# Cyan4973/FiniteStateEntropy

Measured on NVIDIA H100. Metric: encode+decode GB/s (uncompressed) per GPU on 32 KB blocks; bit-exact vs ref, higher is better.
Workload: dtype u8

## Files before the change

### finitestateentropy_b200/csrc/huf_encode.cu

```cuda
#include <cstdlib>
#include <mutex>
#include <vector>
#include "common.cuh"
#include "launch_util.cuh"
#include "fse_dev.cuh"
#include "sink_dev.cuh"
#include "huf_build_dev.cuh"

namespace fseb {
namespace hufe {

constexpr unsigned FULL = 0xFFFFFFFFu;

struct __align__(16) Plan {
    u32 ctable[256];
    u8  header[136];
    u32 hSize;
    u32 state;
    u32 total;
    u32 streamOff[4];
    u32 streamBytes[4];
};

constexpr int PLAN_WARPS = 8;
struct PlanWarp {
    u32   count4[4][256];
    u32   count[256];
    HNode nodes[2 * 256 + 2];
    u32   ctable[256];
    u32   firstVal[32];
    u8    lenOf[256];
    alignas(4) u8 header[136];
};
static_assert(sizeof(HNode) * (2 * 256 + 2) >= 384 * sizeof(u32), "header scratch must fit in the node array");
__device__ __forceinline__ u32 seg_count(const PlanWarp& w, u32 k, u32 i) { return w.count4[k][i]; }

__device__ __forceinline__ void warp_hist_range(u32* cnt, const u8* s, u32 begin, u32 end, unsigned lane)
{
    u32 i = begin;
    u32 const head = min(end, (u32)((begin + 15) & ~15u));
    bool const vec = ((reinterpret_cast<u64>(s) & 15) == 0);
    if (vec) {
        for (u32 k = i + lane; k < head; k += 32) atomicAdd(&cnt[s[k]], 1u);
        i = head;
        u32 const nvec = (end - i) / 16;
        const uint4* const gv = reinterpret_cast<const uint4*>(s + i);
        for (u32 v0 = 0; v0 < nvec; v0 += 128) {
            uint4 x[4];
            #pragma unroll
            for (int h = 0; h < 4; h++) { u32 const vi = v0 + 32 * h + lane; x[h] = (vi < nvec) ? __ldg(gv + vi) : make_uint4(0, 0, 0, 0); }
            #pragma unroll
            for (int h = 0; h < 4; h++) {
                if (v0 + 32 * h + lane >= nvec) continue;
                u32 const wd[4] = { x[h].x, x[h].y, x[h].z, x[h].w };
                #pragma unroll
                for (int k = 0; k < 4; k++) {
                    u32 const y = wd[k];
                    atomicAdd(&cnt[y & 0xFF], 1u); atomicAdd(&cnt[__byte_perm(y, 0, 0x4441)], 1u);
                    atomicAdd(&cnt[__byte_perm(y, 0, 0x4442)], 1u); atomicAdd(&cnt[y >> 24], 1u);
                }
            }
        }
        i += nvec * 16;
    }
    for (u32 k = i + lane; k < end; k += 32) atomicAdd(&cnt[s[k]], 1u);
}

__device__ __forceinline__ void warp_hist4_pipelined(u32 (*count4)[256], const u8* s, u32 n, u32 seg, unsigned lane)
{
    const uint4* const gv = reinterpret_cast<const uint4*>(s) + lane;
    u32 const B = n / 2048, perSeg = seg / 2048;
    auto load = [&](uint4 (&x)[4], u32 b) {
        #pragma unroll
        for (int h = 0; h < 4; h++) x[h] = __ldg(gv + b * 128 + 32 * h);
    };
    auto count = [&](const uint4 (&x)[4], u32 b) {
        u32* const cnt = count4[b / perSeg];
        #pragma unroll
        for (int h = 0; h < 4; h++) {
            u32 const wd[4] = { x[h].x, x[h].y, x[h].z, x[h].w };
            #pragma unroll
            for (int k = 0; k < 4; k++) {
                u32 const y = wd[k];
                atomicAdd(&cnt[y & 0xFF], 1u); atomicAdd(&cnt[__byte_perm(y, 0, 0x4441)], 1u);
                atomicAdd(&cnt[__byte_perm(y, 0, 0x4442)], 1u); atomicAdd(&cnt[y >> 24], 1u);
            }
        }
    };
    uint4 xa[4], xb[4];
    load(xa, 0);
    #pragma unroll 1
    for (u32 b = 0; b < B; b += 2) {
        if (b + 1 < B) load(xb, b + 1);
        count(xa, b);
        if (b + 2 < B) load(xa, b + 2);
        if (b + 1 < B) count(xb, b + 1);
    }
}

__global__ void __launch_bounds__(32 * PLAN_WARPS)
huf_plan_kernel(BatchGeom g, u8* __restrict__ cbuf, u64* __restrict__ csizes, const u8* __restrict__ src,
                unsigned msvReq, unsigned tlogReq, Plan* __restrict__ plans, int serialHeader)
{
    extern __shared__ __align__(16) unsigned char smem_raw[];
    PlanWarp& w = reinterpret_cast<PlanWarp*>(smem_raw)[threadIdx.x >> 5];
    unsigned const lane = threadIdx.x & 31u;
    u32 const b = blockIdx.x * PLAN_WARPS + (threadIdx.x >> 5);
    if (b >= g.nBlocks) return;
    u32 const n = block_len(g, b);
    const u8* const s = src + (u64)b * g.blockSize;
    u8* const d = cbuf + (u64)b * g.slot;
    u64 const cap = g.slot;
    Plan& P = plans[b];
#define FSEB_FINAL(v) do { if (lane == 0) { P.state = 1; csizes[b] = (v); } return; } while (0)

    if (!n) FSEB_FINAL(0);
    if (!cap) FSEB_FINAL(0);
    if (n > HUF_BLOCK_MAX) FSEB_FINAL(err(E_SRC_WRONG));
    if (tlogReq > HUF_MAX_TLOG) FSEB_FINAL(err(E_TLOG_TOO_LARGE));
    if (msvReq > HUF_MAX_SV) FSEB_FINAL(err(E_MSV_TOO_LARGE));
    unsigned const msvDecl = msvReq ? msvReq : HUF_MAX_SV;
    unsigned huffLog = tlogReq ? tlogReq : HUF_DEF_TLOG;

    u32 const seg = (n + 3) / 4;
    for (u32 i = lane; i < 4 * 256; i += 32) (&w.count4[0][0])[i] = 0;
    __syncwarp();
    if ((reinterpret_cast<u64>(s) & 15) == 0 && seg % 2048 == 0 && n == 4 * seg) warp_hist4_pipelined(w.count4, s, n, seg, lane);
    else {
        #pragma unroll 1
        for (u32 k = 0; k < 4; k++) {
            u32 const beg = min(k * seg, n), end = (k < 3) ? min((k + 1) * seg, n) : n;
            warp_hist_range(w.count4[k], s, beg, end, lane);
        }
    }
    __syncwarp();
    u32 top = 0, best = 0;
    for (u32 i = lane; i < 256; i += 32) {
        u32 const c = seg_count(w, 0, i) + seg_count(w, 1, i) + seg_count(w, 2, i) + seg_count(w, 3, i);
        w.count[i] = c;
        if (c) top = i; best = c > best ? c : best;
    }
    #pragma unroll
    for (int dlt = 16; dlt; dlt >>= 1) { top = max(top, __shfl_xor_sync(FULL, top, dlt)); best = max(best, __shfl_xor_sync(FULL, best, dlt)); }
    __syncwarp();
    if (msvDecl < 255 && top > msvDecl) FSEB_FINAL(err(E_MSV_TOO_SMALL));
    if (best == n) { if (lane == 0) d[0] = s[0]; FSEB_FINAL(1); }
    if (best <= (n >> 7) + 4) FSEB_FINAL(0);
    u32 const msv = top;

    huffLog = d_optimal_tablelog(huffLog, n, msv, 1);
    {   u64 const mb = warp_huf_build_ctable(w.ctable, w.count, msv, huffLog, w.nodes, w.lenOf, w.firstVal);
        if (is_err(mb)) FSEB_FINAL(mb);
        huffLog = (u32)mb;
    }
    __syncwarp();
    u32* const wksp = reinterpret_cast<u32*>(w.nodes);
    u64 hs = 0;
    if (serialHeader) { if (lane == 0) hs = d_huf_write_ctable(w.header, cap < sizeof(w.header) ? cap : sizeof(w.header), w.ctable, msv, huffLog, wksp); hs = __shfl_sync(FULL, hs, 0); }
    else hs = warp_huf_write_ctable(w.header, cap < sizeof(w.header) ? cap : sizeof(w.header), w.ctable, msv, huffLog, wksp);
    if (is_err(hs)) FSEB_FINAL(hs);
    if (hs + 12 >= n) FSEB_FINAL(0);
    u64 const capLeft = cap - hs;
    if (capLeft < 6 + 1 + 1 + 1 + 8 || n < 12) FSEB_FINAL(0);
    u32 bits[4];
    #pragma unroll
    for (int k = 0; k < 4; k++) {
        u32 acc = 0;
        for (u32 i = lane; i <= msv; i += 32) acc += seg_count(w, k, i) * (w.ctable[i] >> 16);
        #pragma unroll
        for (int dlt = 16; dlt; dlt >>= 1) acc += __shfl_xor_sync(FULL, acc, dlt);
        bits[k] = acc;
    }
    u64 op = 6; bool fits = true;
    u32 offs[4], lens[4];
    #pragma unroll
    for (int t = 0; t < 4; t++) {
        u64 const capk = capLeft - op;
        u64 const tot = (u64)bits[t] + 1;
        if (fits && (capk <= 8 || (tot >> 3) >= capk - 8)) fits = false;
        offs[t] = (u32)(hs + op); lens[t] = (u32)((tot + 7) >> 3);
        op += lens[t];
    }
    u64 const total = hs + op;
    if (!fits || total >= (u64)n - 1) FSEB_FINAL(0);
    __syncwarp();
    for (u32 i = lane; i < 256; i += 32) P.ctable[i] = w.ctable[i];
    for (u32 i = lane; i < (u32)hs; i += 32) P.header[i] = w.header[i];
    if (lane < 4) { P.streamOff[lane] = offs[lane]; P.streamBytes[lane] = lens[lane]; }
    if (lane == 0) { P.hSize = (u32)hs; P.state = 0; P.total = (u32)total; csizes[b] = total; }
#undef FSEB_FINAL
}

constexpr int THREADS = 128;

__device__ __noinline__ void store_piece_exact(u32* gw, u32 j, uint4 v, u32 a0, u32 endByte)
{
    u32 const wd[4] = { v.x, v.y, v.z, v.w };
    u8* const pb = reinterpret_cast<u8*>(gw + j);
    for (u32 t = 0; t < 16; t++) { u32 const at = 4 * j + t; if (at >= a0 && at < endByte) pb[t] = (u8)(wd[t >> 2] >> (8 * (t & 3))); }
}

__global__ void __launch_bounds__(THREADS)
huf_emit_kernel(BatchGeom g, u8* __restrict__ cbuf, const u8* __restrict__ src, const Plan* __restrict__ plans, const u32* __restrict__ sharedCT)
{
    constexpr u32 W = 512;
    __shared__ u32 ctab[256];
    constexpr u32 WP = W + 4;
    __shared__ __align__(16) u32 winAll[4 * WP];
    int const tid = threadIdx.x;
    unsigned const lane = tid & 31u; int const k = tid >> 5;
    u32 const b = blockIdx.x;
    const Plan& P = plans[b];
    if (P.state != 0) return;
    u32 const n = block_len(g, b);
    const u8* const s = src + (u64)b * g.blockSize;
    u8* const d = cbuf + (u64)b * g.slot;
    u32 const hSize = P.hSize, total = P.total;

    {   const u32* const ct = sharedCT ? sharedCT : P.ctable;
        u32 const c0 = ct[tid], c1 = ct[tid + 128];
        ctab[tid] = (c0 >> 16) | (c0 << 8 & 0xFFFF00u); ctab[tid + 128] = (c1 >> 16) | (c1 << 8 & 0xFFFF00u);
    }
    for (u32 i = tid; i < 4 * WP; i += THREADS) winAll[i] = 0;
    for (u32 i = tid; i < hSize; i += THREADS) d[i] = P.header[i];
    if (tid < 3) { u32 const v = P.streamBytes[tid]; d[hSize + 2 * tid] = (u8)v; d[hSize + 2 * tid + 1] = (u8)(v >> 8); }
    __syncthreads();
    {
        u32 const seg = (n + 3) / 4;
        int const segBeg = (int)(k * seg);
        int const segEnd = (k < 3) ? (int)((k + 1) * seg) : (int)n;
        u32 sTab = (u32)__cvta_generic_to_shared(ctab);
        asm volatile("mov.u32 %0, %0;" : "+r"(sTab));
        u32* const win = winAll + k * WP;
        u32 sWin = (u32)__cvta_generic_to_shared(win);
        asm volatile("mov.u32 %0, %0;" : "+r"(sWin));
        u8* const gstart = d + P.streamOff[k];
        u32 const a0 = (u32)(reinterpret_cast<u64>(gstart) & 15);
        u32* const gw = reinterpret_cast<u32*>(gstart - a0);
        u32 const sBytes = (k < 3) ? P.streamBytes[k] : total - P.streamOff[3];
        u32 const endByte = a0 + sBytes;
        u32 bitpos = 8u * a0;
        u32 flushed = 0;
        auto lds32 = [&](u32 a) -> u32 { u32 v; asm volatile("ld.shared.u32 %0, [%1];" : "=r"(v) : "r"(a)); return v; };
        auto lds64 = [&](u32 o) -> uint2 { u32 const e = lds32(sTab + (o >> 1)); return make_uint2(e >> 8, e & 0xFFu); };
        auto red_or = [&](u32 a, u32 v) { asm volatile("red.shared.or.b32 [%0], %1;" :: "r"(a), "r"(v) : "memory"); };
        auto red_or3 = [&](u32 a, u32 v0, u32 v1, u32 v2) {
            asm volatile("red.shared.or.b32 [%0], %1; red.shared.or.b32 [%0+4], %2; red.shared.or.b32 [%0+8], %3;" :: "r"(a), "r"(v0), "r"(v1), "r"(v2) : "memory");
        };
        auto scan = [&](u32 held, u32& excl) -> u32 {
            u32 incl = held;
            #pragma unroll
            for (int dd = 1; dd < 32; dd <<= 1)
                asm volatile("{ .reg .pred p; .reg .u32 t; shfl.sync.up.b32 t|p, %0, %1, 0, 0xffffffff; @p add.u32 %0, %0, t; }" : "+r"(incl) : "r"(dd));
            excl = incl - held;
            return __shfl_sync(FULL, incl, 31);
        };
        auto put = [&](u32 at, u32 x0, u32 x1) {
            u32 const sh = at & 31;
            red_or3(sWin + ((at >> 3) & (4 * (W - 1))), x0 << sh, __funnelshift_l(x0, x1, sh), __funnelshift_l(x1, 0, sh));
        };
        auto put96 = [&](u32 at, u32 z0, u32 z1, u32 z2) {
            u32 const sh = at & 31;
            asm volatile("red.shared.or.b32 [%0], %1; red.shared.or.b32 [%0+4], %2; red.shared.or.b32 [%0+8], %3; red.shared.or.b32 [%0+12], %4;"
                         :: "r"(sWin + ((at >> 3) & (4 * (W - 1)))), "r"(z0 << sh), "r"(__funnelshift_l(z0, z1, sh)), "r"(__funnelshift_l(z1, z2, sh)),
                            "r"(__funnelshift_l(z2, 0, sh)) : "memory");
        };
        auto flush = [&](bool all) {
            u32 const upTo = all ? (endByte + 3) / 4 : (bitpos >> 5);
            if (!all && flushed + 128 > upTo) return;
            __syncwarp();
            while (all ? flushed < upTo : flushed + 128 <= upTo) {
                u32 const j = flushed + 4 * lane;
                if (j < upTo) {
                    u32 const i = j & (W - 1);
                    uint4 v = *reinterpret_cast<uint4*>(win + i);
                    *reinterpret_cast<uint4*>(win + i) = make_uint4(0, 0, 0, 0);
                    if (i == 0) { v.x |= win[W]; v.y |= win[W + 1]; v.z |= win[W + 2]; win[W] = 0; win[W + 1] = 0; win[W + 2] = 0; }
                    if (!all && (j != 0 || a0 == 0)) *reinterpret_cast<uint4*>(gw + j) = v;
                    else store_piece_exact(gw, j, v, a0, endByte);
                }
                flushed += 128;
            }
        };
        auto place = [&](u32 x0, u32 x1, u32 held) -> u32 {
            u32 excl; u32 const sum = scan(held, excl);
            put(bitpos + excl, x0, x1);
            return sum;
        };
        constexpr int PF = 4;
        int hiCur = segEnd;
        {
            bool const al8 = ((reinterpret_cast<u64>(s) + (u64)segEnd) & 7) == 0;
            int const nBig = al8 ? (segEnd - segBeg) / 256 : 0;
            const uint2* gq = reinterpret_cast<const uint2*>(s + segEnd) - 1 - lane;
            auto half = [&](u32 w, u32& a0, u32& a1) -> u32 {
                u32 const e0 = lds32(sTab + 4 * __byte_perm(w, 0, 0x4443)), e1 = lds32(sTab + 4 * __byte_perm(w, 0, 0x4442));
                u32 const e2 = lds32(sTab + 4 * __byte_perm(w, 0, 0x4441)), e3 = lds32(sTab + 4 * __byte_perm(w, 0, 0x4440));
                u32 const p01 = (e0 >> 8) | __funnelshift_l(0, e1 >> 8, e0), l01 = e0 + e1;
                u32 const p23 = (e2 >> 8) | __funnelshift_l(0, e3 >> 8, e2), l23 = e2 + e3;
                a0 = p01 | __funnelshift_l(0, p23, l01); a1 = __funnelshift_l(p23, 0, l01);
                return (l01 + l23) & 0xFFu;
            };
            auto merge = [&](u32 x0, u32 x1, u32 lx, u32 y0, u32 y1, u32& z0, u32& z1, u32& z2) {
                u32 const t0 = __funnelshift_l(0, y0, lx), t1 = __funnelshift_l(y0, y1, lx), t2 = __funnelshift_l(y1, 0, lx);
                bool const far = (lx & 32u) != 0;
                z0 = x0 | (far ? 0u : t0); z1 = x1 | (far ? t0 : t1); z2 = far ? t1 : t2;
            };
            auto big2 = [&](uint2 curA, uint2 curB) {
                u32 x0, x1, y0, y1, za0, za1, za2, zb0, zb1, zb2;
                u32 lx = half(curA.y, x0, x1), ly = half(curA.x, y0, y1);
                merge(x0, x1, lx, y0, y1, za0, za1, za2);
                u32 const la = lx + ly;
                lx = half(curB.y, x0, x1); ly = half(curB.x, y0, y1);
                merge(x0, x1, lx, y0, y1, zb0, zb1, zb2);
                u32 const lb = lx + ly;
                u32 excl; u32 const sum = scan(la | (lb << 16), excl);
                u32 const sumA = sum & 0xFFFFu;
                put96(bitpos + (excl & 0xFFFFu), za0, za1, za2);
                put96(bitpos + sumA + (excl >> 16), zb0, zb1, zb2);
                bitpos += sumA + (sum >> 16);
                flush(false);
            };
            constexpr int PB = 2;
            int const rounds = nBig / PB;
            uint2 bufA[PB], bufB[PB];
            #pragma unroll
            for (int i = 0; i < PB; i++) { bufA[i] = rounds > 0 ? __ldg(gq - 32 * i) : make_uint2(0, 0); bufB[i] = make_uint2(0, 0); }
            auto round = [&](uint2 (&X)[PB], uint2 (&Y)[PB], int r) {
                gq -= 32 * PB;
                uint2 const c0 = X[0], c1 = X[1];
                if (r + 1 < rounds) { Y[0] = __ldg(gq); Y[1] = __ldg(gq - 32); }
                big2(c0, c1);
            };
            int r = 0;
            #pragma unroll 1
            for (; r + 1 < rounds; r += 2) { round(bufA, bufB, r); round(bufB, bufA, r + 1); }
            if (r < rounds) round(bufA, bufB, r);
            hiCur -= 256 * rounds * PB;
        }
        bool const wordAligned = ((reinterpret_cast<u64>(s) + (u64)hiCur) & 3) == 0;
        int const nFull = wordAligned ? (hiCur - segBeg) / 128 : 0;
        {
            const u32* gp = reinterpret_cast<const u32*>(s + hiCur) - 1 - lane;
            auto group = [&](u32 o0, u32 o1, u32 o2, u32 o3) {
                uint2 const e0 = lds64(o0), e1 = lds64(o1), e2 = lds64(o2), e3 = lds64(o3);
                u32 const p01 = e0.x | (e1.x << e0.y), l01 = e0.y + e1.y;
                u32 const p23 = e2.x | (e3.x << e2.y), l23 = e2.y + e3.y;
                u32 const a0 = p01 | (p23 << l01), a1 = __funnelshift_l(p23, 0, l01);
                bitpos += place(a0, a1, l01 + l23);
                flush(false);
            };
            int const rounds = nFull / PF;
            u32 bufA[PF], bufB[PF];
            #pragma unroll
            for (int i = 0; i < PF; i++) { bufA[i] = rounds > 0 ? __ldg(gp - 32 * i) : 0u; bufB[i] = 0u; }
            auto round = [&](u32 (&X)[PF], u32 (&Y)[PF], int r) {
                gp -= 32 * PF;
                bool const more = r + 1 < rounds;
                #pragma unroll
                for (int i = 0; i < PF; i++) {
                    u32 const cur = X[i];
                    if (more) Y[i] = __ldg(gp - 32 * i);
                    group(8 * (cur >> 24), 8 * __byte_perm(cur, 0, 0x4442), 8 * __byte_perm(cur, 0, 0x4441), 8 * (cur & 0xFFu));
                }
            };
            int r = 0;
            #pragma unroll 1
            for (; r + 1 < rounds; r += 2) { round(bufA, bufB, r); round(bufB, bufA, r + 1); }
            if (r < rounds) round(bufA, bufB, r);
            for (int j = rounds * PF; j < nFull; j++) {
                u32 const cur = __ldg(reinterpret_cast<const u32*>(s + hiCur) - 1 - lane - 32 * j);
                group(8 * (cur >> 24), 8 * __byte_perm(cur, 0, 0x4442), 8 * __byte_perm(cur, 0, 0x4441), 8 * (cur & 0xFFu));
            }
        }
        {
            int const rest = hiCur - 128 * nFull;
            auto fetch = [&](int hi) -> u32 {
                int const top = hi - 4 * (int)lane;
                u32 v = 0;
                if (top - 4 >= segBeg && ((reinterpret_cast<u64>(s + top) & 3) == 0)) v = __ldg(reinterpret_cast<const u32*>(s + top - 4));
                else if (top > segBeg) {
                    #pragma unroll
                    for (int j = 0; j < 4; j++) { int const i = top - 1 - j; if (i >= segBeg) v |= (u32)s[i] << (8 * (3 - j)); }
                }
                return v;
            };
            #pragma unroll 1
            for (int hi = rest; hi > segBeg; hi -= 128) {
                u32 const cur = fetch(hi);
                int const nValid = hi - 4 * (int)lane - segBeg;
                u64 acc = 0; u32 held = 0;
                #pragma unroll
                for (int j = 0; j < 4; j++) {
                    uint2 const e = lds64(8 * ((cur >> (8 * (3 - j))) & 0xFF));
                    if (j < nValid) { acc |= (u64)e.x << held; held += e.y; }
                }
                bitpos += place((u32)acc, (u32)(acc >> 32), held);
                flush(false);
            }
        }
        if (lane == 0) red_or(sWin + 4 * ((bitpos >> 5) & (W - 1)), 1u << (bitpos & 31));
        bitpos += 1;
        flush(true);
    }
}

__global__ void __launch_bounds__(32 * PLAN_WARPS)
huf_sizes_kernel(BatchGeom g, u64* __restrict__ csizes, const u8* __restrict__ src, const u32* __restrict__ ct, Plan* __restrict__ plans)
{
    __shared__ u8 nbOf[256];
    unsigned const lane = threadIdx.x & 31u;
    for (u32 i = threadIdx.x; i < 256; i += blockDim.x) nbOf[i] = (u8)(ct[i] >> 16);
    __syncthreads();
    u32 const b = blockIdx.x * PLAN_WARPS + (threadIdx.x >> 5);
    if (b >= g.nBlocks) return;
    u32 const n = block_len(g, b);
    const u8* const s = src + (u64)b * g.blockSize;
    u64 const cap = g.slot;
    Plan& P = plans[b];
    if (cap < 6 + 1 + 1 + 1 + 8 || n < 12) { if (lane == 0) { P.state = 1; csizes[b] = 0; } return; }
    u32 const seg = (n + 3) / 4;
    u32 bits[4];
    #pragma unroll 1
    for (u32 k = 0; k < 4; k++) {
        u32 const beg = k * seg, end = (k < 3) ? (k + 1) * seg : n;
        u32 acc = 0;
        u32 i = beg + lane * 4;
        if ((reinterpret_cast<u64>(s + beg) & 3) == 0) {
            for (; i + 4 <= end; i += 128) {
                u32 const w = __ldg(reinterpret_cast<const u32*>(s + i));
                acc += nbOf[w & 0xFF] + nbOf[(w >> 8) & 0xFF] + nbOf[(w >> 16) & 0xFF] + nbOf[w >> 24];
            }
            for (u32 t = i; t < end && t < i + 4; t++) acc += nbOf[s[t]];
        } else for (u32 t = beg + lane; t < end; t += 32) acc += nbOf[s[t]];
        #pragma unroll
        for (int dlt = 16; dlt; dlt >>= 1) acc += __shfl_xor_sync(FULL, acc, dlt);
        bits[k] = acc;
    }
    u64 op = 6; bool fits = true;
    u32 offs[4], lens[4];
    #pragma unroll
    for (int t = 0; t < 4; t++) {
        u64 const capk = cap - op;
        u64 const tot = (u64)bits[t] + 1;
        if (fits && (capk <= 8 || (tot >> 3) >= capk - 8)) fits = false;
        offs[t] = (u32)op; lens[t] = (u32)((tot + 7) >> 3);
        op += lens[t];
    }
    if (!fits) { if (lane == 0) { P.state = 1; csizes[b] = 0; } return; }
    if (lane < 4) { P.streamOff[lane] = offs[lane]; P.streamBytes[lane] = lens[lane]; }
    if (lane == 0) { P.hSize = 0; P.state = 0; P.total = (u32)op; csizes[b] = op; }
}

}

cudaError_t launch_huf_encode_using_ctable(const BatchGeom& g, void* cbuf, u64* csizes, const void* src, const u32* dCTable, cudaStream_t stream)
{
    if (g.nBlocks == 0) return cudaSuccess;
    cudaError_t e;
    hufe::Plan* const plans = (hufe::Plan*)stream_scratch(2, stream, sizeof(hufe::Plan) * (size_t)g.nBlocks, &e);
    if (e != cudaSuccess) return e;
    unsigned const grid = (g.nBlocks + hufe::PLAN_WARPS - 1) / hufe::PLAN_WARPS;
    hufe::huf_sizes_kernel<<<grid, 32 * hufe::PLAN_WARPS, 0, stream>>>(g, csizes, (const u8*)src, dCTable, plans);
    hufe::huf_emit_kernel<<<g.nBlocks, hufe::THREADS, 0, stream>>>(g, (u8*)cbuf, (const u8*)src, plans, dCTable);
    return cudaGetLastError();
}

cudaError_t launch_huf_encode(const BatchGeom& g, void* cbuf, u64* csizes, const void* src,
                              unsigned msv, unsigned tlog, cudaStream_t stream)
{
    if (g.nBlocks == 0) return cudaSuccess;
    cudaError_t e;
    hufe::Plan* plans = nullptr;
    static int asyncScratch = -1;
    if (asyncScratch < 0) { const char* const v = getenv("FSEB200_SCRATCH_ASYNC"); asyncScratch = (v && atoi(v) == 1) ? 1 : 0; }
    size_t const need = sizeof(hufe::Plan) * (size_t)g.nBlocks;
    if (asyncScratch) e = cudaMallocAsync((void**)&plans, need, stream);
    else {
        struct Slot { int dev; cudaStream_t s; void* p; size_t cap; };
        static std::mutex mu; static std::vector<Slot> slots;
        std::lock_guard<std::mutex> lock(mu);
        int dev = 0; cudaGetDevice(&dev);
        Slot* hit = nullptr;
        for (auto& sl : slots) if (sl.s == stream && sl.dev == dev) { hit = &sl; break; }
        if (!hit) { slots.push_back(Slot{ dev, stream, nullptr, 0 }); hit = &slots.back(); }
        e = cudaSuccess;
        if (hit->cap < need) {
            if (hit->p) { cudaStreamSynchronize(stream); cudaFree(hit->p); hit->p = nullptr; hit->cap = 0; }
            e = cudaMalloc(&hit->p, need);
            if (e == cudaSuccess) hit->cap = need;
        }
        plans = (hufe::Plan*)hit->p;
    }
    if (e != cudaSuccess) return e;
    static int serialHeader = -1;
    if (serialHeader < 0) { const char* const v = getenv("FSEB200_HUF_SERIAL_HEADER"); serialHeader = (v && atoi(v) == 1) ? 1 : 0; }
    static u32 const subBatch = [] { const char* const v = getenv("FSEB200_HUF_ENC_SUBBATCH"); long n = v ? atol(v) : 0; return (u32)(n < 0 ? 0 : n); }();
    size_t const smem = sizeof(hufe::PlanWarp) * hufe::PLAN_WARPS;
    static SmemOptIn optin;
    e = optin.ensure(hufe::huf_plan_kernel, current_device(), (int)smem);
    if (e != cudaSuccess) return e;
    u32 const step = (subBatch && subBatch < g.nBlocks) ? subBatch : g.nBlocks;
    for (u32 b0 = 0; b0 < g.nBlocks; b0 += step) {
        BatchGeom gs = g;
        gs.nBlocks = (g.nBlocks - b0 < step) ? g.nBlocks - b0 : step;
        u64 const off = (u64)b0 * g.blockSize;
        u64 const span = (u64)gs.nBlocks * g.blockSize;
        gs.total = (g.total - off < span) ? g.total - off : span;
        u8* const cb = (u8*)cbuf + (u64)b0 * g.slot; const u8* const sp = (const u8*)src + off;
        unsigned const grid = (gs.nBlocks + hufe::PLAN_WARPS - 1) / hufe::PLAN_WARPS;
        hufe::huf_plan_kernel<<<grid, 32 * hufe::PLAN_WARPS, smem, stream>>>(gs, cb, csizes + b0, sp, msv, tlog, plans + b0, serialHeader);
        hufe::huf_emit_kernel<<<gs.nBlocks, hufe::THREADS, 0, stream>>>(gs, cb, sp, plans + b0, nullptr);
    }
    e = cudaGetLastError();
    cudaError_t const e2 = asyncScratch ? cudaFreeAsync(plans, stream) : cudaSuccess;
    return e != cudaSuccess ? e : e2;
}

}
```

Measured before the change: 380.3.

## Overlap Huffman plan and emit kernels via programmatic launch and per-block ready flags

The plan kernel now triggers dependent launch early, and the emit kernel is launched with programmatic stream serialization. Each emit block spins on a per-block release/acquire ready flag until its plan is published, so emit work can start while planning is still running. Plan warps per CTA drop from 8 to 4, giving smaller CTAs that finish more evenly, and the sizes kernel keeps its own 8-warp constant. The cost is a memset of the flags, spin-waiting emit CTAs that occupy SM slots, and a deadlock risk if emit CTAs take all residency before the plan CTAs are scheduled.

New measurement: 388.7, median of 6. +2.2%, better.

```diff
diff --git a/finitestateentropy_b200/csrc/huf_encode.cu b/finitestateentropy_b200/csrc/huf_encode.cu
--- a/finitestateentropy_b200/csrc/huf_encode.cu
+++ b/finitestateentropy_b200/csrc/huf_encode.cu
@@ -22,7 +22,7 @@
     u32 streamBytes[4];
 };
 
-constexpr int PLAN_WARPS = 8;
+constexpr int PLAN_WARPS = 4;
 struct PlanWarp {
     u32   count4[4][256];
     u32   count[256];
@@ -33,6 +33,8 @@
     alignas(4) u8 header[136];
 };
 static_assert(sizeof(HNode) * (2 * 256 + 2) >= 384 * sizeof(u32), "header scratch must fit in the node array");
+__device__ __forceinline__ void publish(u32* flag) { asm volatile("st.release.gpu.global.u32 [%0], 1;" :: "l"(flag) : "memory"); }
+__device__ __forceinline__ u32 published(const u32* flag) { u32 v; asm volatile("ld.acquire.gpu.global.u32 %0, [%1];" : "=r"(v) : "l"(flag) : "memory"); return v; }
 __device__ __forceinline__ u32 seg_count(const PlanWarp& w, u32 k, u32 i) { return w.count4[k][i]; }
 
 __device__ __forceinline__ void warp_hist_range(u32* cnt, const u8* s, u32 begin, u32 end, unsigned lane)
@@ -100,8 +102,9 @@
 
 __global__ void __launch_bounds__(32 * PLAN_WARPS)
 huf_plan_kernel(BatchGeom g, u8* __restrict__ cbuf, u64* __restrict__ csizes, const u8* __restrict__ src,
-                unsigned msvReq, unsigned tlogReq, Plan* __restrict__ plans, int serialHeader)
-{
+                unsigned msvReq, unsigned tlogReq, Plan* __restrict__ plans, u32* __restrict__ ready, int serialHeader)
+{
+    asm volatile("griddepcontrol.launch_dependents;");
     extern __shared__ __align__(16) unsigned char smem_raw[];
     PlanWarp& w = reinterpret_cast<PlanWarp*>(smem_raw)[threadIdx.x >> 5];
     unsigned const lane = threadIdx.x & 31u;
@@ -112,7 +115,7 @@
     u8* const d = cbuf + (u64)b * g.slot;
     u64 const cap = g.slot;
     Plan& P = plans[b];
-#define FSEB_FINAL(v) do { if (lane == 0) { P.state = 1; csizes[b] = (v); } return; } while (0)
+#define FSEB_FINAL(v) do { if (lane == 0) { P.state = 1; csizes[b] = (v); __threadfence(); publish(ready + b); } return; } while (0)
 
     if (!n) FSEB_FINAL(0);
     if (!cap) FSEB_FINAL(0);
@@ -188,6 +191,9 @@
     for (u32 i = lane; i < (u32)hs; i += 32) P.header[i] = w.header[i];
     if (lane < 4) { P.streamOff[lane] = offs[lane]; P.streamBytes[lane] = lens[lane]; }
     if (lane == 0) { P.hSize = (u32)hs; P.state = 0; P.total = (u32)total; csizes[b] = total; }
+    __threadfence();
+    __syncwarp();
+    if (lane == 0) publish(ready + b);
 #undef FSEB_FINAL
 }
 
@@ -201,7 +207,7 @@
 }
 
 __global__ void __launch_bounds__(THREADS)
-huf_emit_kernel(BatchGeom g, u8* __restrict__ cbuf, const u8* __restrict__ src, const Plan* __restrict__ plans, const u32* __restrict__ sharedCT)
+huf_emit_kernel(BatchGeom g, u8* __restrict__ cbuf, const u8* __restrict__ src, const Plan* plans, const u32* ready, const u32* __restrict__ sharedCT)
 {
     constexpr u32 W = 512;
     __shared__ u32 ctab[256];
@@ -210,6 +216,10 @@
     int const tid = threadIdx.x;
     unsigned const lane = tid & 31u; int const k = tid >> 5;
     u32 const b = blockIdx.x;
+    if (ready) {
+        if (tid == 0) while (!published(ready + b)) __nanosleep(200);
+        __syncthreads();
+    }
     const Plan& P = plans[b];
     if (P.state != 0) return;
     u32 const n = block_len(g, b);
@@ -405,14 +415,15 @@
     }
 }
 
-__global__ void __launch_bounds__(32 * PLAN_WARPS)
+constexpr int SIZES_WARPS = 8;
+__global__ void __launch_bounds__(32 * SIZES_WARPS)
 huf_sizes_kernel(BatchGeom g, u64* __restrict__ csizes, const u8* __restrict__ src, const u32* __restrict__ ct, Plan* __restrict__ plans)
 {
     __shared__ u8 nbOf[256];
     unsigned const lane = threadIdx.x & 31u;
     for (u32 i = threadIdx.x; i < 256; i += blockDim.x) nbOf[i] = (u8)(ct[i] >> 16);
     __syncthreads();
-    u32 const b = blockIdx.x * PLAN_WARPS + (threadIdx.x >> 5);
+    u32 const b = blockIdx.x * SIZES_WARPS + (threadIdx.x >> 5);
     if (b >= g.nBlocks) return;
     u32 const n = block_len(g, b);
     const u8* const s = src + (u64)b * g.blockSize;
@@ -460,9 +471,9 @@
     cudaError_t e;
     hufe::Plan* const plans = (hufe::Plan*)stream_scratch(2, stream, sizeof(hufe::Plan) * (size_t)g.nBlocks, &e);
     if (e != cudaSuccess) return e;
-    unsigned const grid = (g.nBlocks + hufe::PLAN_WARPS - 1) / hufe::PLAN_WARPS;
-    hufe::huf_sizes_kernel<<<grid, 32 * hufe::PLAN_WARPS, 0, stream>>>(g, csizes, (const u8*)src, dCTable, plans);
-    hufe::huf_emit_kernel<<<g.nBlocks, hufe::THREADS, 0, stream>>>(g, (u8*)cbuf, (const u8*)src, plans, dCTable);
+    unsigned const grid = (g.nBlocks + hufe::SIZES_WARPS - 1) / hufe::SIZES_WARPS;
+    hufe::huf_sizes_kernel<<<grid, 32 * hufe::SIZES_WARPS, 0, stream>>>(g, csizes, (const u8*)src, dCTable, plans);
+    hufe::huf_emit_kernel<<<g.nBlocks, hufe::THREADS, 0, stream>>>(g, (u8*)cbuf, (const u8*)src, plans, nullptr, dCTable);
     return cudaGetLastError();
 }
 
@@ -474,7 +485,7 @@
     hufe::Plan* plans = nullptr;
     static int asyncScratch = -1;
     if (asyncScratch < 0) { const char* const v = getenv("FSEB200_SCRATCH_ASYNC"); asyncScratch = (v && atoi(v) == 1) ? 1 : 0; }
-    size_t const need = sizeof(hufe::Plan) * (size_t)g.nBlocks;
+    size_t const need = (sizeof(hufe::Plan) + sizeof(u32)) * (size_t)g.nBlocks;
     if (asyncScratch) e = cudaMallocAsync((void**)&plans, need, stream);
     else {
         struct Slot { int dev; cudaStream_t s; void* p; size_t cap; };
@@ -492,6 +503,9 @@
         }
         plans = (hufe::Plan*)hit->p;
     }
+    if (e != cudaSuccess) return e;
+    u32* const ready = reinterpret_cast<u32*>(plans + g.nBlocks);
+    e = cudaMemsetAsync(ready, 0, sizeof(u32) * (size_t)g.nBlocks, stream);
     if (e != cudaSuccess) return e;
     static int serialHeader = -1;
     if (serialHeader < 0) { const char* const v = getenv("FSEB200_HUF_SERIAL_HEADER"); serialHeader = (v && atoi(v) == 1) ? 1 : 0; }
@@ -509,8 +523,14 @@
         gs.total = (g.total - off < span) ? g.total - off : span;
         u8* const cb = (u8*)cbuf + (u64)b0 * g.slot; const u8* const sp = (const u8*)src + off;
         unsigned const grid = (gs.nBlocks + hufe::PLAN_WARPS - 1) / hufe::PLAN_WARPS;
-        hufe::huf_plan_kernel<<<grid, 32 * hufe::PLAN_WARPS, smem, stream>>>(gs, cb, csizes + b0, sp, msv, tlog, plans + b0, serialHeader);
-        hufe::huf_emit_kernel<<<gs.nBlocks, hufe::THREADS, 0, stream>>>(gs, cb, sp, plans + b0, nullptr);
+        hufe::huf_plan_kernel<<<grid, 32 * hufe::PLAN_WARPS, smem, stream>>>(gs, cb, csizes + b0, sp, msv, tlog, plans + b0, ready + b0, serialHeader);
+        cudaLaunchConfig_t cfg = {};
+        cfg.gridDim = dim3(gs.nBlocks); cfg.blockDim = dim3(hufe::THREADS); cfg.stream = stream;
+        cudaLaunchAttribute attr[1];
+        attr[0].id = cudaLaunchAttributeProgrammaticStreamSerialization; attr[0].val.programmaticStreamSerializationAllowed = 1;
+        cfg.attrs = attr; cfg.numAttrs = 1;
+        e = cudaLaunchKernelEx(&cfg, hufe::huf_emit_kernel, gs, cb, sp, (const hufe::Plan*)(plans + b0), (const u32*)(ready + b0), (const u32*)nullptr);
+        if (e != cudaSuccess) break;
     }
     e = cudaGetLastError();
     cudaError_t const e2 = asyncScratch ? cudaFreeAsync(plans, stream) : cudaSuccess;
```
